# linchaobao/EPPM

Measured on AMD Instinct MI355X. Metric: Mflow-vectors/sec, higher is better.
Workload: dtype f32; 1 GPU; single 1024x436 Sintel-shape synthetic pair per step, full 3-level pyramid, patch_r=9, default defs.h parameters; 1 rank(s), independent pairs; inputs: RGBA planes resident in HBM before the timed region; outputs: interleaved float2 flow left in HBM (the PCIe-inclusive window of the reference API -- host RGB in, host u/v out -- is `host_boundary`, with --full); inputs=device-resident RGBA, outputs=device-resident float2 flow, pairs_in_flight_per_gpu=24, pairs_per_launch=8, contexts_in_flight=3, width=1024, height=436

## Files before the change

eppm_amd/csrc/c2f_device.cuh:

```cuda
#pragma once
#include "eppm_device.cuh"

#ifndef EPPM_C2F_UNROLL
#define EPPM_C2F_UNROLL 2
#endif
#ifndef EPPM_C2F_WAVES
#define EPPM_C2F_WAVES 4
#endif
#ifndef EPPM_C2F_WAVES_MIN
#define EPPM_C2F_WAVES_MIN 2
#endif
#define EPPM_C2F_OCC __attribute__((amdgpu_waves_per_eu(EPPM_C2F_WAVES_MIN, EPPM_C2F_WAVES)))
#ifndef EPPM_C2F_WIN_H
#ifdef EPPM_TOL
#define EPPM_C2F_WIN_H 50
#else
#define EPPM_C2F_WIN_H 48
#endif
#endif
#ifndef EPPM_C2F_PASS2
#define EPPM_C2F_PASS2 1
#endif
#ifndef EPPM_C2F_WIN_WAVES
#define EPPM_C2F_WIN_WAVES 4
#endif
#ifndef EPPM_C2F_PRE
#define EPPM_C2F_PRE 1
#endif
#ifndef EPPM_C2F_PRE_ROWS
#define EPPM_C2F_PRE_ROWS 5
#endif
#ifndef EPPM_C2F_PRE_EPS
#define EPPM_C2F_PRE_EPS 0x1p-13f
#endif
#define EPPM_C2F_PRE_DMIN 0x1p-60f
#define EPPM_C2F_PRE_RHSMIN 0x1p-100f
#ifndef EPPM_C2F_SPLIT_BELOW_WAVES
#define EPPM_C2F_SPLIT_BELOW_WAVES 1024
#endif
#ifndef EPPM_C2F_WINDOW
#define EPPM_C2F_WINDOW 1
#endif
#ifndef EPPM_C2F_WINDOW17
#define EPPM_C2F_WINDOW17 1
#endif
#ifdef EPPM_TOL
#define EPPM_C2F_LOG2 true
#else
#define EPPM_C2F_LOG2 false
#endif
#define EPPM_PRAGMA_(x) _Pragma(#x)
#define EPPM_UNROLL(n) EPPM_PRAGMA_(unroll n)

namespace eppm {

__device__ __forceinline__ Planes to_dev(const PlanesH& h, size_t pstride = 0, unsigned pair = 0)
{
    Planes p;
    p.pk1 = pair_ptr((const float4*)h.pk1, pstride, pair); p.pk2 = pair_ptr((const float4*)h.pk2, pstride, pair);
    p.w = h.w; p.h = h.h; p.pitch = h.pitch;
    return p;
}

__device__ __forceinline__ float4 stage_texel(const uint32_t* __restrict__ pc, const float4* __restrict__ pk, unsigned idx)
{
    if (pc) { const uint32_t w = pc[idx]; return make_texel(w, w >> 24); }
    return pk[idx];
}

__device__ __forceinline__ bool c2f_unknown(float fvx, float fvy) { return fvx > kUnknownFlowThresh || fvy > kUnknownFlowThresh; }
__device__ __forceinline__ int c2f_centre(float f, int x) { return (int)(int16_t)(f2short(f) + x); }
__device__ __forceinline__ void c2f_store_flow(float* flow, int idx, int fx, int fy)
{
    flow[idx * 2] = (float)fx;
    flow[idx * 2 + 1] = (float)fy;
}
__device__ __forceinline__ float c2f_min(float a, float b) { return (a < b) ? a : b; }
__device__ __forceinline__ float c2f_min4(float c1, float c2, float c3, float c4) { return c2f_min(c1, c2f_min(c2, c2f_min(c3, c4))); }
template <class F>
__device__ __forceinline__ void c2f_select_best(float* flow, int x, int y, int ccx, int ccy, int w, int h, F cost_of)
{
    int bx = ccx, by = ccy;
    float min_cost = 999999;
#pragma unroll
    for (int m = 0; m < 3; m++) {
        const int cx = (int)(int16_t)(ccx + m - 1);
        if (cx < 0 || cx >= w) continue;
#pragma unroll
        for (int n = 0; n < 3; n++) {
            const int cy = (int)(int16_t)(ccy + n - 1);
            if (cy < 0 || cy >= h) continue;
            const float cv = cost_of(m, n);
            if (cv < min_cost) { min_cost = cv; bx = cx; by = cy; }
        }
    }
    flow[(y * w + x) * 2] = (float)(bx - x);
    flow[(y * w + x) * 2 + 1] = (float)(by - y);
}

template <int SPLIT>
__device__ __forceinline__ bool c2f_tile_origin(const Planes& P, int& x0, int& y0, int& part)
{
    const int tiles_x = (P.w + kBlock - 1) / kBlock, tiles = tiles_x * ((P.h + kBlock - 1) / kBlock);
    const int per_xcd = (tiles + 7) / 8;
    const int slot = SPLIT ? (blockIdx.x >> 3) / SPLIT : (blockIdx.x >> 3);
    part = SPLIT ? (blockIdx.x >> 3) % SPLIT : -1;
    const int tile = (blockIdx.x & 7) * per_xcd + slot;
    if (slot >= per_xcd || tile >= tiles) return false;
    x0 = (tile % tiles_x) * kBlock; y0 = (tile / tiles_x) * kBlock;
    return true;
}

template <int R> struct C2fSrcTile { static constexpr int TWU = kBlock + 2 * R, TW = (TWU + 15) / 16 * 16; };
template <int R> struct C2fPreList {
    static constexpr int PADB = (C2fSrcTile<R>::TW - C2fSrcTile<R>::TWU) * 16, KROWS = PADB ? (256 * 8 + PADB - 1) / PADB : 0;
    static constexpr int CAP = PADB ? (C2fSrcTile<R>::TWU - KROWS) * (PADB / 2) : 0;
// ... 298 lines not shown
```

eppm_amd/csrc/eppm_internal.h:

```cpp
#pragma once

#include <hip/hip_runtime.h>
#include <stddef.h>
#include <stdint.h>

#include <atomic>

#include "../../include/eppm.h"

namespace eppm {

constexpr int kMaxLevels = 8;
constexpr int kNumLevels = 3;
constexpr int kBlock = 16;
constexpr int kMaxS = 32;
constexpr int kWmfRadius = 4;
constexpr int kBlfRadius = 10;
constexpr int kDeltaSlots = 800;

struct Batch {
    int n;
    size_t stride;
};
constexpr Batch kOnePair = {1, 0};
// ... 57 lines not shown
    int npairs = 1;
    size_t stride = 0;
    size_t cache_plane = 0;
    int wl_units = 0;
    int sweep_seq = 0;
    size_t seed_plane = 0;
    int merged_it = 0;
    int seg_len = 0, nseg_row = 0, nseg_col = 0;
};
int pm_worklist_units(int w, int h, int seg_len);
inline size_t pm_worklist_words(int w, int h, int seg_len) { return 16 + 10 * (size_t)pm_worklist_units(w, h, seg_len); }
struct PmRngDev {
    const uint32_t* init_tab;
    const uint32_t* iter_tab;
    const uint32_t* skip_mat;
    uint32_t skip_weyl;
    int per_lane;
    int gx, gy;
    const int16_t* rand_tab = nullptr;
};
void launch_pm_rand_table(const PmRngDev& rng, uint32_t* work, int16_t* tab, int G, hipStream_t s);
void launch_pm_init_field(const PmBatch& b, const PmRngDev& rng, hipStream_t s);
void launch_pm_cost_field(const PmBatch& b, const float* lut, int R, hipStream_t s);
int pm_parity_kernels(int R);
bool launch_pm_sweep(PmBatch& b, const float* lut, int R, int seg_len, int dir, hipStream_t s, bool speculative = false);
bool launch_pm_sweeps_merged(PmBatch& b, const float* lut, int R, int seg_len, int iteration, hipStream_t s);
void launch_pm_jump(const PmBatch& b, const float* lut, int R, int step, hipStream_t s);
void launch_pm_neighbor(const PmBatch& b, const float* lut, int R, hipStream_t s);
void launch_pm_random_search(const PmBatch& b, const PmRngDev& rng, const float* lut, int R, int search_range, int num_guess,
                             hipStream_t s, bool pretest = false);
void launch_pm_rest_weight(const PmBatch& b, const float* lut, int R, hipStream_t s);
bool pm_search_pretest_ready(const PmBatch& b, const PmRngDev& rng, int R);
struct PmPretestSums { float* n[2]; float* d[2]; };
void launch_pm_pretest_probe(const PmBatch& b, const float* lut, int R, const PmPretestSums& out, hipStream_t s);
EPPM_DECISION bool pm_search_pretest_form(int w, int h, int R, int problems, int npairs);
EPPM_DECISION bool pm_search_pretest(int iteration, int w, int h, int R, int problems, int npairs);
EPPM_DECISION void pm_search_pretest_knobs(int R, int* row0, int* rows, int* from, float* eps);
EPPM_DECISION int pm_search_rows(int w, int h, int R, int problems, int npairs, bool table);
struct SweepForm { int lpc; bool small, pre, tile; };
EPPM_DECISION SweepForm pm_sweep_form(int w, int h, int R, int seg_len, int dir, int problems, int npairs);

struct PmSeed {
    const int16_t* prior[2];
    int16_t* nnf_init[2];
    float* cost_init[2];
    size_t stride = 0;
};
void launch_pm_cost_select(const PmBatch& b, const PmSeed& seed, const float* lut, int R, hipStream_t s);

constexpr int kTemporalMaxSlots = 4096;
struct TemporalArgs {
    const int16_t* prev[2];
    int16_t* prior[2];
    int32_t* keys[2];
    int step[2];
    int w, h, ndir;
    int nslots;
    size_t stride;
    uint32_t armed[kTemporalMaxSlots / 32];
};
void launch_temporal_keys_init(int32_t* keys, int n, hipStream_t s);
void launch_temporal_splat(const TemporalArgs& a, hipStream_t s);
void launch_temporal_gather(const TemporalArgs& a, hipStream_t s);
void launch_temporal_snapshot(int16_t* prev, size_t prev_stride, const int16_t* nnf, int nnf_pitch, int w, int h, hipStream_t s, Batch bt = kOnePair);
void launch_nnf2flow_snapshot(float* flow, int flow_pitch, int16_t* prev, size_t prev_stride, const int16_t* nnf, int nnf_pitch, int w, int h,
                              hipStream_t s, Batch bt = kOnePair);

void launch_lr_check(int16_t* nnf1, float* cost1, const int16_t* nnf2, int w, int h, int cost_pitch, int nnf_pitch, hipStream_t s, Batch bt = kOnePair);
void launch_outlier(int16_t* nnf_out, float* cost, const int16_t* nnf_in, int w, int h, int cost_pitch, int nnf_pitch, hipStream_t s, Batch bt = kOnePair);
size_t wmf_workspace_words(int w, int h, int num_iter);
int16_t* launch_wmf(int16_t* buf_a, int16_t* buf_b, const uint32_t* img, int ipitch, int w, int h, int nnf_pitch,
                    const float* wmf_lut, int num_iter, int only_occlusion, uint32_t* ws, hipStream_t s, Batch bt = kOnePair);
void launch_fill_holes(int16_t* nnf_out, const int16_t* nnf_in, const uint32_t* img, int ipitch, int w, int h, int nnf_pitch,
                       hipStream_t s, Batch bt = kOnePair);
void launch_nnf2flow(float* flow, int flow_pitch, const int16_t* nnf, int nnf_pitch, int w, int h, hipStream_t s, Batch bt = kOnePair);

void launch_resize_flow(float* out, int outH, int outW, const float* in, int h, int w, float ratio, float post_scale, hipStream_t s, Batch bt = kOnePair);
void launch_mul_scalar(float* flow, float scale, int h, int w, hipStream_t s);
EPPM_DECISION int c2f_refine_split_factor(int w, int h, int R, int npairs = 1, bool no_split = false);
bool c2f_refine_wants_split(int w, int h, int R, int npairs = 1, bool no_split = false);
bool c2f_window_span(int R, int* span_x, int* span_y);
void launch_c2f_refine(const PlanesH& P, float* flow, const float* lut, int R, float* cost9, hipStream_t s, Batch bt = kOnePair, bool no_split = false,
                       int pre = -1, unsigned* stat = nullptr, float* probe = nullptr);
void c2f_pretest_knobs(int R, int* on, int* row0, int* rows, int* cap, float* eps, float* dmin, float* rhsmin);
void launch_flow_blf(float* out, const float* in, const uint32_t* img, int ipitch, int w, int h, int flow_pitch,
                     const float* blf_lut, hipStream_t s, Batch bt = kOnePair);
EPPM_DECISION int flow_blf_pixels_per_lane(int w, int h, int npairs = 1);
void launch_flow_jbu(float* out, const float* in_coarse, const uint32_t* img, int ipitch, int w, int h, int wc, int hc, const float* blf_lut,
                     hipStream_t s, Batch bt = kOnePair);

void launch_split_flow(float* uv, const float* flow, int n, hipStream_t s, Batch bt = kOnePair);

void launch_fb_occlusion(uint8_t* occ1, uint8_t* occ2, const float* fwd, size_t fwd_stride, const float* bwd, size_t bwd_stride, int h, int w,
                         float alpha, float beta, int npairs, int ndir, hipStream_t s);

constexpr int kInterpChunk = 4;
struct InterpArgs {
    const uint8_t* img1;
    const uint8_t* img2;
    size_t img_pitch, img_stride;
    const float* flow;
    size_t flow_stride;
    const uint8_t* occ1;
    const uint8_t* occ2;
    size_t occ_stride;
    uint64_t* keys;
    int32_t* fill1;
    int32_t* fill2;
    size_t plane;
    uint8_t* rgb;
    uint8_t* rgba[kInterpChunk];
    size_t rgba_pitch;
    int h, w, nt;
    float t[kInterpChunk];
};
void launch_interp_splat(const InterpArgs& a, int npairs, hipStream_t s);
void launch_interp_fill(const InterpArgs& a, int npairs, hipStream_t s);
void launch_interp_blend(const InterpArgs& a, int npairs, hipStream_t s);

struct MBlurArgs {
    const uint8_t* img;
    size_t img_pitch, img_stride;
    const float* flow;
    size_t flow_stride;
    uint32_t* packed;
    uint64_t* tkeys;
    size_t plane, tplane;
    uint8_t* rgb;
    uint8_t* rgba;
    size_t rgba_pitch;
    int h, w, tiles_x, tiles_y;
    float shutter, max_radius;
    int taps;
};
void launch_mblur_pack(const MBlurArgs& a, int npairs, hipStream_t s);
void launch_mblur_gather(const MBlurArgs& a, int npairs, hipStream_t s);

enum {
    kTrackCntLive, kTrackCntNextId, kTrackCntFrame, kTrackCntDropped, kTrackCntEnded, kTrackCntSeeded,
    kTrackCntIdBase, kTrackCntSurv, kTrackCntPrevLive, kTrackCntSeeded0, kTrackCntDropped0, kTrackCntN = 16
};
struct TrackRec;
struct TrackDev {
    struct {
        int spacing;
        long long min_eig;
        float fb_alpha, fb_beta, mb_alpha, mb_beta;
    } p;
    int cap, ncells, ncx;
    float* npos;
    uint8_t* stat;
    TrackRec* ended;
    int32_t* ended_reason;
    uint8_t* cov;
    uint8_t* flags;
    int32_t *blk_s, *blk_e;
    int32_t* blk_c;
    int32_t* cnt;
};
struct TrackIn {
    const uint8_t* img1;
    const uint8_t* img2;
    size_t pitch;
    const float* fwd;
    const float* bwd;
    int h, w;
};
// ... 195 lines not shown
```

eppm_amd/csrc/k_c2f_refine.hip:

```cpp
#include <type_traits>

#include "c2f_device.cuh"
#include "eppm_internal.h"

namespace eppm {

__constant__ C2fTables<9> c2f_tab9 = make_c2f_tables<9>();
__constant__ C2fTables<17> c2f_tab17 = make_c2f_tables<17>();
template <> __device__ __forceinline__ const C2fTables<9>& c2f_tables<9>() { return c2f_tab9; }
template <> __device__ __forceinline__ const C2fTables<17>& c2f_tables<17>() { return c2f_tab17; }

__global__ __launch_bounds__(256) void k_c2f_refine(PlanesH Ph, float* __restrict__ flow_, const float* __restrict__ lut, int R, size_t pstride)
{
    __shared__ EPPM_LUT_ALIGN PatchLut L;
    load_patch_lut(L, lut, R, threadIdx.y * kBlock + threadIdx.x, 256);
    __syncthreads();
    const Planes P = to_dev(Ph, pstride, blockIdx.z);
    float* __restrict__ flow = pair_ptr(flow_, pstride, blockIdx.z);
    const int x = blockIdx.x * kBlock + threadIdx.x, y = blockIdx.y * kBlock + threadIdx.y;
    if (x >= P.w || y >= P.h) return;
    const float fvx = flow[(y * P.w + x) * 2], fvy = flow[(y * P.w + x) * 2 + 1];
    if (c2f_unknown(fvx, fvy)) { c2f_store_flow(flow, y * P.w + x, 0, 0); return; }
    const int ccx = c2f_centre(fvx, x), ccy = c2f_centre(fvy, y);
    int bx = ccx, by = ccy;
// ... 19 lines not shown
{
    float* __restrict__ flow = pair_ptr(flow_, pstride, blockIdx.y);
    float* __restrict__ cost9 = pair_ptr_opt(cost9_, pstride, blockIdx.y);
    constexpr int TWU = C2fSrcTile<R>::TWU, TW = C2fSrcTile<R>::TW;
    __shared__ EPPM_LUT_ALIGN PatchLutT<R + 1> L;
    __shared__ float4 s_src[TWU * TW];
    const int tid = threadIdx.y * kBlock + threadIdx.x;
    load_patch_lut<EPPM_C2F_LOG2>(L, lut, R, tid, 256);
    const Planes P = to_dev(Ph, pstride, blockIdx.y);
    int x0, y0, part;
    if (!c2f_tile_origin<SPLIT>(P, x0, y0, part)) return;
    const int m_only = (SPLIT == 3) ? part : -1;
    for (int t = tid; t < TWU * TWU; t += 256) {
        const int ry = t / TWU, rx = t % TWU;
        const int sy = iclamp(y0 + ry - R, 0, P.h - 1), sx = iclamp(x0 + rx - R, 0, P.w - 1);
        s_src[ry * TW + rx] = P.pk1[(unsigned)(sy * P.pitch + sx)];
    }
    __syncthreads();
    const int x = x0 + threadIdx.x, y = y0 + threadIdx.y;
    if (x >= P.w || y >= P.h) return;
    const float fvx = flow[(y * P.w + x) * 2], fvy = flow[(y * P.w + x) * 2 + 1];
    if (c2f_unknown(fvx, fvy)) {
        if (SPLIT == 0) c2f_store_flow(flow, y * P.w + x, 0, 0);
        return;
    }
    const int ccx = c2f_centre(fvx, x), ccy = c2f_centre(fvy, y);
    const rgbf c1 = texel_rgb(s_src[(threadIdx.y + R) * TW + threadIdx.x + R]);
    int bx = ccx, by = ccy;
    float min_cost = 999999;
#pragma unroll 1
    for (int m = 0; m < 3; m++) {
        if (SPLIT == 3 && m != m_only) continue;
        const int cx = (int)(int16_t)(ccx + m - 1);
        if (cx < 0 || cx >= P.w) continue;
        rgbf c2[3];
#pragma unroll
        for (int n = 0; n < 3; n++) c2[n] = texel_rgb(tex_px(P.pk2, P.pitch, P.w, P.h, cx, ccy + n - 1));
        float run[3];
        const int cx16 = cx << 4, wmax16 = (P.w - 1) << 4;
        if (SPLIT == 4) {
            if (part == 3) c2f_pass<R, 3, true>(P, L, s_src, TW, threadIdx.x, threadIdx.y, cx16, wmax16, ccy, c1, c2, run);
            else if (part == 2) c2f_pass<R, 2, true>(P, L, s_src, TW, threadIdx.x, threadIdx.y, cx16, wmax16, ccy, c1, c2, run);
            else if (part == 1) c2f_pass<R, 1, true>(P, L, s_src, TW, threadIdx.x, threadIdx.y, cx16, wmax16, ccy, c1, c2, run);
            else c2f_pass<R, 0, true>(P, L, s_src, TW, threadIdx.x, threadIdx.y, cx16, wmax16, ccy, c1, c2, run);
#pragma unroll
            for (int n = 0; n < 3; n++) cost9[(size_t)(y * P.w + x) * 36 + part * 9 + m * 3 + n] = run[n];
            continue;
        }
        c2f_pass<R, 3>(P, L, s_src, TW, threadIdx.x, threadIdx.y, cx16, wmax16, ccy, c1, c2, run);
        c2f_pass<R, 2>(P, L, s_src, TW, threadIdx.x, threadIdx.y, cx16, wmax16, ccy, c1, c2, run);
        c2f_pass<R, 1>(P, L, s_src, TW, threadIdx.x, threadIdx.y, cx16, wmax16, ccy, c1, c2, run);
        c2f_pass<R, 0>(P, L, s_src, TW, threadIdx.x, threadIdx.y, cx16, wmax16, ccy, c1, c2, run);
        if (SPLIT == 3) {
#pragma unroll
            for (int n = 0; n < 3; n++) cost9[(size_t)(y * P.w + x) * 36 + m * 3 + n] = run[n];
            continue;
        }
#pragma unroll
        for (int n = 0; n < 3; n++) {
            const int cy = (int)(int16_t)(ccy + n - 1);
            if (cy < 0 || cy >= P.h) continue;
            const float cv = run[n];
            if (cv < min_cost) { min_cost = cv; bx = cx; by = cy; }
        }
    }
    if (SPLIT != 0) return;
    flow[(y * P.w + x) * 2] = (float)(bx - x);
    flow[(y * P.w + x) * 2 + 1] = (float)(by - y);
}

template <int R, bool PROBE = false>
__global__ __launch_bounds__(512) __attribute__((amdgpu_waves_per_eu(EPPM_C2F_WIN_WAVES, EPPM_C2F_WIN_WAVES)))
void k_c2f_refine_win(PlanesH Ph, float* __restrict__ flow_, const float* __restrict__ lut, size_t pstride, int pre, unsigned* __restrict__ stat,
                      float* __restrict__ probe)
{
    using W = C2fWinShape<R>;
    constexpr int TWU = C2fSrcTile<R>::TWU, TW = C2fSrcTile<R>::TW, WW = W::WW, WH = W::WH;
    static_assert(TWU * TW * 16 >= 9 * 256 * 4, "the exchange buffer aliases the source tile");
    __shared__ EPPM_LUT_ALIGN PatchLutT<R + 1> L;
    __shared__ float4 s_src[TWU * TW];
    __shared__ float4 s_win[WH * WW];
    __shared__ int s_mm[4];
#ifndef EPPM_TOL
    __shared__ int s_pre[8];
#endif
    float* __restrict__ flow = pair_ptr(flow_, pstride, blockIdx.y);
    const int ptid = threadIdx.y * kBlock + threadIdx.x;
    const int grp = threadIdx.z;
    const int tid = grp * 256 + ptid;
    load_patch_lut<EPPM_C2F_LOG2>(L, lut, R, tid, 512);
    const Planes P = to_dev(Ph, pstride, blockIdx.y);
    const uint32_t* __restrict__ pc1 = pair_ptr_opt(Ph.pc1, pstride, blockIdx.y);
    const uint32_t* __restrict__ pc2 = pair_ptr_opt(Ph.pc2, pstride, blockIdx.y);
    int x0, y0, part;
    if (!c2f_tile_origin<0>(P, x0, y0, part)) return;
    if (tid == 0) { s_mm[0] = 0x7fffffff; s_mm[1] = -0x7fffffff; s_mm[2] = 0x7fffffff; s_mm[3] = -0x7fffffff; }
#ifndef EPPM_TOL
    if (tid < 8) s_pre[tid] = 0;
#endif
    for (int t = tid; t < TWU * TWU; t += 512) {
        const int ry = t / TWU, rx = t % TWU;
        const int sy = iclamp(y0 + ry - R, 0, P.h - 1), sx = iclamp(x0 + rx - R, 0, P.w - 1);
        s_src[ry * TW + rx] = stage_texel(pc1, P.pk1, (unsigned)(sy * P.pitch + sx));
    }
    __syncthreads();
    const int x = x0 + threadIdx.x, y = y0 + threadIdx.y;
    const bool inimg = (x < P.w && y < P.h);
    float fvx = 0.0f, fvy = 0.0f;
    if (inimg) { fvx = flow[(y * P.w + x) * 2]; fvy = flow[(y * P.w + x) * 2 + 1]; }
    const bool known = inimg && !(fvx > kUnknownFlowThresh || fvy > kUnknownFlowThresh);
    const int ccx = c2f_centre(fvx, x), ccy = c2f_centre(fvy, y);
    if (known && grp == 0) {
        atomicMin(&s_mm[0], ccx); atomicMax(&s_mm[1], ccx);
        atomicMin(&s_mm[2], ccy); atomicMax(&s_mm[3], ccy);
    }
    __syncthreads();
    const int mnx = s_mm[0], mxx = s_mm[1], mny = s_mm[2], mxy = s_mm[3];
    const bool coherent = (mxx - mnx <= W::SPAN_X) && (mxy - mny <= W::SPAN_Y);
    const int wx0 = mnx - 1 + W::XLO, wy0 = mny - 1 + W::YLO;
    if (coherent && mxx >= mnx) {
        for (int t = tid; t < WH * WW; t += 512) {
            const int sy = iclamp(wy0 + t / WW, 0, P.h - 1), sx = iclamp(wx0 + t % WW, 0, P.w - 1);
            s_win[t] = stage_texel(pc2, P.pk2, (unsigned)(sy * P.pitch + sx));
        }
    }
    __syncthreads();
#ifndef EPPM_TOL
    int path = 3;
    if (pre && coherent && mxx >= mnx) {
        constexpr int S = R + 1, I0 = (S - EPPM_C2F_PRE_ROWS) / 2, I1 = I0 + EPPM_C2F_PRE_ROWS;
        constexpr int PADB = C2fPreList<R>::PADB, KROWS = C2fPreList<R>::KROWS, CAP = C2fPreList<R>::CAP;
        static_assert(PADB % 8 == 0 && PADB > 0 && KROWS < TWU, "keys and items do not straddle a row's padding");
        auto pad = [&](int o) -> char* { return reinterpret_cast<char*>(s_src) + (o / PADB) * (TW * 16) + TWU * 16 + (o % PADB); };
        auto key_at = [&](int p) -> unsigned long long* { return reinterpret_cast<unsigned long long*>(pad(p * 8)); };
        auto item_at = [&](int i) -> uint16_t* { return reinterpret_cast<uint16_t*>(pad(KROWS * PADB + i * 2)); };
        const int lane = tid & 63;
        float N[18], D[18], U = 0.0f;
        unsigned vmask = 0;
        rgbf c1 = {0.0f, 0.0f, 0.0f};
        if (known) {
            c1 = texel_rgb(s_src[(threadIdx.y + R) * TW + threadIdx.x + R]);
#pragma unroll 1
            for (int ii = 0; ii < S; ii++) {
                if (ii >= I0 && ii < I1) continue;
                const float4* __restrict__ srow = s_src + (threadIdx.y + 2 * ii) * TW + threadIdx.x;
#pragma unroll
                for (int jj = 0; jj < S; jj++) U += rest_weight_term(c1, srow[2 * jj], L.gsp[ii * S + jj]);
            }
        }
#pragma unroll
        for (int m = 0; m < 3; m++) {
            const int cx = (int)(int16_t)(ccx + m - 1);
            float cs[6] = {0.0f, 0.0f, 0.0f, 0.0f, 0.0f, 0.0f}, ws[6] = {0.0f, 0.0f, 0.0f, 0.0f, 0.0f, 0.0f};
            if (known && !(cx < 0 || cx >= P.w)) {
                const int wbase = ((ccy - 1 - wy0) * WW + (cx - wx0)) * 16;
                rgbf c2[3];
#pragma unroll
                for (int n = 0; n < 3; n++) {
                    c2[n] = texel_rgb(*reinterpret_cast<const float4*>(reinterpret_cast<const char*>(s_win) + wbase + n * (WW * 16)));
                    const int cy = (int)(int16_t)(ccy + n - 1);
                    if (!(cy < 0 || cy >= P.h)) vmask |= 1u << (m * 3 + n);
                }
                if (grp == 0) c2f_rows2_win<R, 3, 2, WW, I0, I1, 3>(L, s_src, TW, threadIdx.x, threadIdx.y, c1, c2, s_win, wbase, cs, ws);
                else c2f_rows2_win<R, 1, 0, WW, I0, I1, 3>(L, s_src, TW, threadIdx.x, threadIdx.y, c1, c2, s_win, wbase, cs, ws);
            }
#pragma unroll
            for (int n = 0; n < 3; n++) { N[m * 3 + n] = cs[n]; D[m * 3 + n] = ws[n]; N[9 + m * 3 + n] = cs[3 + n]; D[9 + m * 3 + n] = ws[3 + n]; }
        }
        if (PROBE && known) {
            float* __restrict__ pp = probe + ((size_t)blockIdx.y * P.h * P.w + (size_t)y * P.w + x) * 73;
            const int qa = (grp == 0 ? 3 : 1) * 9, qb = (grp == 0 ? 2 : 0) * 9;
#pragma unroll
            for (int k = 0; k < 9; k++) { pp[qa + k] = N[k]; pp[36 + qa + k] = D[k]; pp[qb + k] = N[9 + k]; pp[36 + qb + k] = D[9 + k]; }
            if (grp == 1) pp[72] = U;
        }
        bool small = false;
#pragma unroll
        for (int k = 0; k < 9; k++)
            if ((vmask >> k) & 1) small = small || !(D[k] > EPPM_C2F_PRE_DMIN) || !(D[9 + k] > EPPM_C2F_PRE_DMIN);
        if (small) s_pre[0] = 1;
        if (grp == 1) {
            int ks = 15;
            float e_best = 0.0f;
#pragma unroll
            for (int k = 0; k < 9; k++) {
                if (!((vmask >> k) & 1)) continue;
                const float e = c2f_min(N[k] / D[k], N[9 + k] / D[9 + k]);
                if (ks == 15 || e < e_best) { e_best = e; ks = k; }
            }
            *key_at(ptid) = 0xfffffffffffffff0ull | (unsigned)ks;
        }
        __syncthreads();
        path = 1;
        if (!s_pre[0]) {
            const int ks = (int)(*reinterpret_cast<const uint32_t*>(key_at(ptid)) & 15u);
            const bool live = known && ks != 15;
            if (live) {
                const int cx = (int)(int16_t)(ccx + ks / 3 - 1);
                const int wbase = ((ccy - 1 + ks % 3 - wy0) * WW + (cx - wx0)) * 16;
                const rgbf c2[1] = {texel_rgb(*reinterpret_cast<const float4*>(reinterpret_cast<const char*>(s_win) + wbase))};
                float cs[2], ws[2];
                if (grp == 0) c2f_rows2_win<R, 3, 2, WW, 0, S, 1>(L, s_src, TW, threadIdx.x, threadIdx.y, c1, c2, s_win, wbase, cs, ws);
                else c2f_rows2_win<R, 1, 0, WW, 0, S, 1>(L, s_src, TW, threadIdx.x, threadIdx.y, c1, c2, s_win, wbase, cs, ws);
                const float c = c2f_min(cs[0] / ws[0], cs[1] / ws[1]);
                atomicMin(key_at(ptid), ((unsigned long long)__float_as_uint(c) << 4) | (unsigned)ks);
            }
            __syncthreads();
            unsigned sa = 0, sb = 0, tested = 0;
            if (live) {
                const float B = __uint_as_float((uint32_t)(*key_at(ptid) >> 4));
#pragma unroll
                for (int k = 0; k < 9; k++) {
                    if (!((vmask >> k) & 1) || k == ks) continue;
                    const float ra = B * (D[k] + U), rb = B * (D[9 + k] + U);
                    if (!(N[k] * (1.0f - EPPM_C2F_PRE_EPS) >= ra && ra >= EPPM_C2F_PRE_RHSMIN)) sa |= 1u << k;
                    if (!(N[9 + k] * (1.0f - EPPM_C2F_PRE_EPS) >= rb && rb >= EPPM_C2F_PRE_RHSMIN)) sb |= 1u << k;
                    tested += 2;
                }
            }
            const int na = __popc(sa), nb = __popc(sb);
            int ia = na, ib = nb;
#pragma unroll
            for (int d = 1; d < 64; d <<= 1) {
                const int ta = __shfl_up(ia, d), tb = __shfl_up(ib, d);
                if (lane >= d) { ia += ta; ib += tb; }
            }
            const int pa = grp == 0 ? 3 : 1, pb = grp == 0 ? 2 : 0;
            int wa = 0, wb = 0;
            if (lane == 63) { wa = atomicAdd(&s_pre[1 + pa], ia); wb = atomicAdd(&s_pre[1 + pb], ib); }
            wa = __shfl(wa, 63); wb = __shfl(wb, 63);
            if (stat && tested) { atomicAdd(stat + 4, tested); atomicAdd(stat + 5, tested - (unsigned)(na + nb)); }
            __syncthreads();
            int cnt[4], chb[5];
            chb[0] = 0;
#pragma unroll
            for (int p = 0; p < 4; p++) { cnt[p] = s_pre[1 + p]; chb[p + 1] = chb[p] + ((cnt[p] + 63) >> 6); }
            path = 2;
            if (chb[4] * 64 <= CAP) {
                path = 0;
                {
                    int at = chb[pa] * 64 + wa + ia - na;
                    for (unsigned s = sa; s; s &= s - 1) *item_at(at++) = (uint16_t)(ptid | ((__ffs(s) - 1) << 8));
                    at = chb[pb] * 64 + wb + ib - nb;
                    for (unsigned s = sb; s; s &= s - 1) *item_at(at++) = (uint16_t)(ptid | ((__ffs(s) - 1) << 8));
                }
                __syncthreads();
                for (int c = tid >> 6; c < chb[4]; c += 8) {
                    const int p = __builtin_amdgcn_readfirstlane((c >= chb[1]) + (c >= chb[2]) + (c >= chb[3]));
                    const int idx = (c - chb[p]) * 64 + lane;
                    if (idx < cnt[p]) {
                        const unsigned it = *item_at(chb[p] * 64 + idx);
                        const int ip = it & 255, k = it >> 8, tx = ip & (kBlock - 1), ty = ip / kBlock;
                        const int px = x0 + tx, py = y0 + ty;
                        const int qcx = c2f_centre(flow[(py * P.w + px) * 2], px), qcy = c2f_centre(flow[(py * P.w + px) * 2 + 1], py);
                        const int cx = (int)(int16_t)(qcx + k / 3 - 1);
                        const int wbase = ((qcy - 1 + k % 3 - wy0) * WW + (cx - wx0)) * 16;
                        const rgbf q1 = texel_rgb(s_src[(ty + R) * TW + tx + R]);
                        const rgbf q2 = texel_rgb(*reinterpret_cast<const float4*>(reinterpret_cast<const char*>(s_win) + wbase));
                        float c_;
                        if (p == 3) c_ = c2f_one_win<R, 3, WW>(L, s_src, TW, tx, ty, q1, q2, s_win, wbase);
                        else if (p == 2) c_ = c2f_one_win<R, 2, WW>(L, s_src, TW, tx, ty, q1, q2, s_win, wbase);
                        else if (p == 1) c_ = c2f_one_win<R, 1, WW>(L, s_src, TW, tx, ty, q1, q2, s_win, wbase);
                        else c_ = c2f_one_win<R, 0, WW>(L, s_src, TW, tx, ty, q1, q2, s_win, wbase);
                        atomicMin(key_at(ip), ((unsigned long long)__float_as_uint(c_) << 4) | (unsigned)k);
                    }
                }
                __syncthreads();
                if (stat && tid == 0) atomicAdd(stat + 0, 1u);
                if (grp != 1 || !inimg) return;
                if (!known) { c2f_store_flow(flow, y * P.w + x, 0, 0); return; }
                int k = (int)(*key_at(ptid) & 15u);
                if (k == 15) k = 4;
                c2f_store_flow(flow, y * P.w + x, (int)(int16_t)(ccx + k / 3 - 1) - x, (int)(int16_t)(ccy + k % 3 - 1) - y);
                return;
            }
        }
    }
    if (stat && tid == 0) atomicAdd(stat + path, 1u);
#endif
    float res[9];
    float res1[9];
    if (known) {
        const rgbf c1 = texel_rgb(s_src[(threadIdx.y + R) * TW + threadIdx.x + R]);
#pragma unroll
        for (int m = 0; m < 3; m++) {
            const int cx = (int)(int16_t)(ccx + m - 1);
            float run[3] = {0.0f, 0.0f, 0.0f}, raw[3] = {0.0f, 0.0f, 0.0f};
            if (!(cx < 0 || cx >= P.w)) {
                rgbf c2[3];
                const int cx16 = cx << 4, wmax16 = (P.w - 1) << 4;
                if (coherent) {
                    const int wbase = ((ccy - 1 - wy0) * WW + (cx - wx0)) * 16;
#pragma unroll
                    for (int n = 0; n < 3; n++) c2[n] = texel_rgb(*reinterpret_cast<const float4*>(reinterpret_cast<const char*>(s_win) + wbase + n * (WW * 16)));
#if EPPM_C2F_PASS2
                    if (grp == 0) {
                        float c4[3], c3[3];
                        c2f_pass2_win<R, 3, 2, WW>(L, s_src, TW, threadIdx.x, threadIdx.y, c1, c2, s_win, wbase, c4, c3);
#pragma unroll
                        for (int n = 0; n < 3; n++) run[n] = c2f_min(c3[n], c4[n]);
                    } else {
                        c2f_pass2_win<R, 1, 0, WW>(L, s_src, TW, threadIdx.x, threadIdx.y, c1, c2, s_win, wbase, run, raw);
                    }
#else
                    if (grp == 0) {
                        c2f_pass<R, 3, false, true, WW>(P, L, s_src, TW, threadIdx.x, threadIdx.y, cx16, wmax16, ccy, c1, c2, run, s_win, wbase);
                        c2f_pass<R, 2, false, true, WW>(P, L, s_src, TW, threadIdx.x, threadIdx.y, cx16, wmax16, ccy, c1, c2, run, s_win, wbase);
                    } else {
                        c2f_pass<R, 1, true, true, WW>(P, L, s_src, TW, threadIdx.x, threadIdx.y, cx16, wmax16, ccy, c1, c2, run, s_win, wbase);
                        c2f_pass<R, 0, true, true, WW>(P, L, s_src, TW, threadIdx.x, threadIdx.y, cx16, wmax16, ccy, c1, c2, raw, s_win, wbase);
                    }
#endif
                } else {
#pragma unroll
                    for (int n = 0; n < 3; n++) c2[n] = texel_rgb(tex_px(P.pk2, P.pitch, P.w, P.h, cx, ccy + n - 1));
                    if (grp == 0) {
                        c2f_pass<R, 3>(P, L, s_src, TW, threadIdx.x, threadIdx.y, cx16, wmax16, ccy, c1, c2, run);
                        c2f_pass<R, 2>(P, L, s_src, TW, threadIdx.x, threadIdx.y, cx16, wmax16, ccy, c1, c2, run);
                    } else {
                        c2f_pass<R, 1, true>(P, L, s_src, TW, threadIdx.x, threadIdx.y, cx16, wmax16, ccy, c1, c2, run);
                        c2f_pass<R, 0, true>(P, L, s_src, TW, threadIdx.x, threadIdx.y, cx16, wmax16, ccy, c1, c2, raw);
                    }
                }
            }
#pragma unroll
            for (int n = 0; n < 3; n++) { res[m * 3 + n] = run[n]; res1[m * 3 + n] = raw[n]; }
        }
    }
    __syncthreads();
    float* __restrict__ xch = reinterpret_cast<float*>(s_src);
    if (grp == 0 && known) {
#pragma unroll
        for (int k = 0; k < 9; k++) xch[k * 256 + ptid] = res[k];
    }
    __syncthreads();
    if (grp != 1 || !inimg) return;
    if (!known) { c2f_store_flow(flow, y * P.w + x, 0, 0); return; }
    int bx = ccx, by = ccy;
    float min_cost = 999999;
#pragma unroll
    for (int m = 0; m < 3; m++) {
        const int cx = (int)(int16_t)(ccx + m - 1);
        if (cx < 0 || cx >= P.w) continue;
#pragma unroll
        for (int n = 0; n < 3; n++) {
            const int cy = (int)(int16_t)(ccy + n - 1);
            if (cy < 0 || cy >= P.h) continue;
            const float m34 = xch[(m * 3 + n) * 256 + ptid];
            const float c_2 = res[m * 3 + n], c_1 = res1[m * 3 + n];
            const float cv = c2f_min(c_1, c2f_min(c_2, m34));
            if (cv < min_cost) { min_cost = cv; bx = cx; by = cy; }
// ... 63 lines not shown
            if (!(cx < 0 || cx >= P.w)) {
                rgbf c2[3];
                const int cx16 = cx << 4, wmax16 = (P.w - 1) << 4;
                if (coherent) {
                    const int wbase = ((ccy - 1 - wy0) * WW + (cx - wx0)) * 16;
#pragma unroll
                    for (int n = 0; n < 3; n++) c2[n] = texel_rgb(*reinterpret_cast<const float4*>(reinterpret_cast<const char*>(s_win) + wbase + n * (WW * 16)));
                    if (grp == 0) c2f_pass<R, 3, true, true, WW>(P, L, s_src, TW, threadIdx.x, threadIdx.y, cx16, wmax16, ccy, c1, c2, run, s_win, wbase);
                    else if (grp == 1) c2f_pass<R, 2, true, true, WW>(P, L, s_src, TW, threadIdx.x, threadIdx.y, cx16, wmax16, ccy, c1, c2, run, s_win, wbase);
                    else if (grp == 2) c2f_pass<R, 1, true, true, WW>(P, L, s_src, TW, threadIdx.x, threadIdx.y, cx16, wmax16, ccy, c1, c2, run, s_win, wbase);
                    else c2f_pass<R, 0, true, true, WW>(P, L, s_src, TW, threadIdx.x, threadIdx.y, cx16, wmax16, ccy, c1, c2, run, s_win, wbase);
                } else {
#pragma unroll
                    for (int n = 0; n < 3; n++) c2[n] = texel_rgb(tex_px(P.pk2, P.pitch, P.w, P.h, cx, ccy + n - 1));
                    if (grp == 0) c2f_pass<R, 3, true>(P, L, s_src, TW, threadIdx.x, threadIdx.y, cx16, wmax16, ccy, c1, c2, run);
                    else if (grp == 1) c2f_pass<R, 2, true>(P, L, s_src, TW, threadIdx.x, threadIdx.y, cx16, wmax16, ccy, c1, c2, run);
                    else if (grp == 2) c2f_pass<R, 1, true>(P, L, s_src, TW, threadIdx.x, threadIdx.y, cx16, wmax16, ccy, c1, c2, run);
                    else c2f_pass<R, 0, true>(P, L, s_src, TW, threadIdx.x, threadIdx.y, cx16, wmax16, ccy, c1, c2, run);
                }
            }
#pragma unroll
            for (int n = 0; n < 3; n++) res[m * 3 + n] = run[n];
        }
    }
    __syncthreads();
    float* __restrict__ xch = reinterpret_cast<float*>(s_src);
    if (grp != 0 && known) {
#pragma unroll
        for (int k = 0; k < 9; k++) xch[((grp - 1) * 9 + k) * 256 + ptid] = res[k];
    }
    __syncthreads();
    if (grp != 0 || !inimg) return;
    if (!known) { c2f_store_flow(flow, y * P.w + x, 0, 0); return; }
    int bx = ccx, by = ccy;
    float min_cost = 999999;
#pragma unroll
    for (int m = 0; m < 3; m++) {
        const int cx = (int)(int16_t)(ccx + m - 1);
        if (cx < 0 || cx >= P.w) continue;
#pragma unroll
        for (int n = 0; n < 3; n++) {
            const int cy = (int)(int16_t)(ccy + n - 1);
            if (cy < 0 || cy >= P.h) continue;
            const int k = m * 3 + n;
            const float c_4 = res[k], c_3 = xch[k * 256 + ptid], c_2 = xch[(9 + k) * 256 + ptid], c_1 = xch[(18 + k) * 256 + ptid];
            const float cv = c2f_min4(c_1, c_2, c_3, c_4);
            if (cv < min_cost) { min_cost = cv; bx = cx; by = cy; }
        }
    }
    flow[(y * P.w + x) * 2] = (float)(bx - x);
    flow[(y * P.w + x) * 2 + 1] = (float)(by - y);
}

template <int SPLIT>
__global__ __launch_bounds__(256) void k_c2f_select(float* __restrict__ flow_, const float* __restrict__ cost9_, int w, int h, size_t pstride)
{
    float* __restrict__ flow = pair_ptr(flow_, pstride, blockIdx.z);
    const float* __restrict__ cost9 = pair_ptr(cost9_, pstride, blockIdx.z);
    const int x = blockIdx.x * blockDim.x + threadIdx.x, y = blockIdx.y * blockDim.y + threadIdx.y;
    if (x >= w || y >= h) return;
    const float fvx = flow[(y * w + x) * 2], fvy = flow[(y * w + x) * 2 + 1];
    if (c2f_unknown(fvx, fvy)) { c2f_store_flow(flow, y * w + x, 0, 0); return; }
    c2f_select_best(flow, x, y, c2f_centre(fvx, x), c2f_centre(fvy, y), w, h, [=](int m, int n) {
        const float* __restrict__ pc = cost9 + (size_t)(y * w + x) * 36 + m * 3 + n;
        float cv = pc[0];
        if (SPLIT == 4) {
            cv = pc[27];
            cv = c2f_min(pc[18], cv);
            cv = c2f_min(pc[9], cv);
            cv = c2f_min(pc[0], cv);
        }
        return cv;
    });
}

bool c2f_window_span(int R, int* span_x, int* span_y)
{
    if (!(R == 9 || R == 17)) return false;
    *span_x = (R == 9) ? C2fWinShape<9>::SPAN_X : C2fWinShape<17>::SPAN_X;
    *span_y = (R == 9) ? C2fWinShape<9>::SPAN_Y : C2fWinShape<17>::SPAN_Y;
    return true;
}

void c2f_pretest_knobs(int R, int* on, int* row0, int* rows, int* cap, float* eps, float* dmin, float* rhsmin)
{
#ifdef EPPM_TOL
    *on = 0;
#else
    *on = EPPM_C2F_PRE;
#endif
    *row0 = (R + 1 - EPPM_C2F_PRE_ROWS) / 2; *rows = EPPM_C2F_PRE_ROWS;
    *cap = C2fPreList<9>::CAP;
    *eps = EPPM_C2F_PRE_EPS; *dmin = EPPM_C2F_PRE_DMIN; *rhsmin = EPPM_C2F_PRE_RHSMIN;
}

static bool c2f_table_ok(int w, int h, int R) { return (w + R < 32764) && (h + R < 32764); }

int c2f_refine_split_factor(int w, int h, int R, int npairs, bool no_split)
{
    if (no_split || !(R == 9 || R == 17) || !c2f_table_ok(w, h, R)) return 0;
    const int tiles = ((w + kBlock - 1) / kBlock) * ((h + kBlock - 1) / kBlock);
    if (!(tiles * npairs * 4 < EPPM_C2F_SPLIT_BELOW_WAVES)) return 0;
    auto imbalance = [&](int f) { const int wgs = tiles * f * npairs; return (float)((wgs + 255) / 256) * 256.0f / (float)wgs; };
    return (imbalance(4) < imbalance(3)) ? 4 : 3;
}
bool c2f_refine_wants_split(int w, int h, int R, int npairs, bool no_split) { return c2f_refine_split_factor(w, h, R, npairs, no_split) != 0; }

template <class F>
static void with_radius(int R, F&& f)
{
    if (R == 9) f(std::integral_constant<int, 9>{});
    else f(std::integral_constant<int, 17>{});
}

void launch_c2f_refine(const PlanesH& P, float* flow, const float* lut, int R, float* cost9, hipStream_t s, Batch bt, bool no_split, int pre,
                       unsigned* stat, float* probe)
{
    dim3 grid((P.w + kBlock - 1) / kBlock, (P.h + kBlock - 1) / kBlock, bt.n), block(kBlock, kBlock);
    const int per_xcd = (grid.x * grid.y + 7) / 8;
    dim3 grid1(per_xcd * 8, bt.n);
    const int f = cost9 ? c2f_refine_split_factor(P.w, P.h, R, bt.n, no_split) : 0;
    launch_note(kLaunchRefine, P.w, P.h, bt.n, f, R);
    if (f) {
        dim3 gridf(per_xcd * f * 8, bt.n), gs((P.w + 63) / 64, (P.h + 3) / 4, bt.n), bs(64, 4);
        with_radius(R, [&](auto r) {
            if (f == 3) hipLaunchKernelGGL((k_c2f_refine_tiled<r(), 3>), gridf, block, 0, s, P, flow, lut, cost9, bt.stride);
            else hipLaunchKernelGGL((k_c2f_refine_tiled<r(), 4>), gridf, block, 0, s, P, flow, lut, cost9, bt.stride);
        });
        if (f == 3) hipLaunchKernelGGL(k_c2f_select<3>, gs, bs, 0, s, flow, cost9, P.w, P.h, bt.stride);
        else hipLaunchKernelGGL(k_c2f_select<4>, gs, bs, 0, s, flow, cost9, P.w, P.h, bt.stride);
        return;
    }
    if (!(R == 9 || R == 17) || !c2f_table_ok(P.w, P.h, R)) {
        hipLaunchKernelGGL(k_c2f_refine, grid, block, 0, s, P, flow, lut, R, bt.stride);
        return;
    }
    const bool window = (R == 9) ? EPPM_C2F_WINDOW : EPPM_C2F_WINDOW17;
    if (!window) with_radius(R, [&](auto r) { hipLaunchKernelGGL((k_c2f_refine_tiled<r(), 0>), grid1, block, 0, s, P, flow, lut, (float*)nullptr, bt.stride); });
    else if (R == 9 && probe) hipLaunchKernelGGL((k_c2f_refine_win<9, true>), grid1, dim3(kBlock, kBlock, 2), 0, s, P, flow, lut, bt.stride, 1, stat, probe);
    else if (R == 9) hipLaunchKernelGGL((k_c2f_refine_win<9>), grid1, dim3(kBlock, kBlock, 2), 0, s, P, flow, lut, bt.stride, pre < 0 ? EPPM_C2F_PRE : pre, stat, (float*)nullptr);
    else hipLaunchKernelGGL((k_c2f_refine_win4<17>), grid1, dim3(kBlock, kBlock, 4), 0, s, P, flow, lut, bt.stride);
}

}
```

eppm_amd/stages.py:

```python
import ctypes as C

import numpy as np

from ._lib import CParams, check, check_launcher, lib, probe_dispatch
from .api import float2, short2, uchar4


class Dev:

    def __init__(self, arr=None, shape=None, dtype=None, pitched=False):
        if arr is not None:
            arr = np.ascontiguousarray(arr)
            shape, dtype = arr.shape, arr.dtype
        self.h, self.w = shape
        self.dtype = np.dtype(dtype)
        row = self.w * self.dtype.itemsize
        self.ptr = C.c_void_p()
        if pitched:
            pitch = C.c_size_t()
            check(lib().eppm_malloc_pitched(C.byref(self.ptr), C.byref(pitch), C.c_size_t(row), C.c_size_t(self.h)), "malloc_pitched")
            self.pitch = pitch.value
        else:
            check(lib().eppm_malloc_device(C.byref(self.ptr), C.c_size_t(row * self.h)), "malloc")
            self.pitch = row
# ... 196 lines not shown
    check(lib().eppm_probe_search_pretest(iteration, w, h, patch_r, problems, npairs, out, C.byref(eps)), "eppm_probe_search_pretest")
    return bool(out[0]), out[1], out[2], out[3], eps.value, bool(out[4])


def patchmatch(P):
    n, c = Dev(shape=(P.h, P.w), dtype=short2), Dev(shape=(P.h, P.w), dtype=np.float32)
    lib().baoCudaPatchMatch(n.ptr, c.ptr, *P.args(), P.w, P.h, _sz(P.i1.pitch), _sz(c.pitch), _sz(n.pitch), _sz(P.c1.pitch))
    check_launcher("baoCudaPatchMatch")
    return n.get(), c.get()


def left_right_check(nnf1, cost1, nnf2, cost2):
    h, w = nnf1.shape
    a, b, c, d = Dev(nnf1), Dev(cost1), Dev(nnf2), Dev(cost2)
    lib().baoCudaLeftRightCheck(a.ptr, b.ptr, c.ptr, d.ptr, w, h, _sz(b.pitch), _sz(a.pitch))
    check_launcher("baoCudaLeftRightCheck")
    return a.get(), b.get(), c.get(), d.get()


def outlier_removal(nnf, cost):
    h, w = nnf.shape
    a, b = Dev(nnf), Dev(cost)
    lib().baoCudaOutlierRemoval(a.ptr, b.ptr, w, h, _sz(b.pitch), _sz(a.pitch))
    check_launcher("baoCudaOutlierRemoval")
    return a.get(), b.get()


def weighted_median(nnf, img, num_iter=20, only_occlusion=True):
    h, w = nnf.shape
    a, i = Dev(nnf), Dev(img, pitched=True)
    lib().baoCudaWeightedMedianFilter(a.ptr, None, i.ptr, w, h, _sz(i.pitch), _sz(w * 4), _sz(a.pitch), num_iter, C.c_bool(only_occlusion))
    check_launcher("baoCudaWeightedMedianFilter")
    return a.get()


def fill_holes(nnf, img):
    h, w = nnf.shape
    a, i = Dev(nnf), Dev(img, pitched=True)
    lib().baoCudaFillHole(a.ptr, None, i.ptr, w, h, _sz(i.pitch), _sz(w * 4), _sz(a.pitch))
    check_launcher("baoCudaFillHole")
    return a.get()


def nnf2flow(nnf):
    h, w = nnf.shape
    a, f = Dev(nnf), Dev(shape=(h, w), dtype=float2)
    lib().baoCudaNNF2Flow(f.ptr, a.ptr, w, h, _sz(a.pitch), _sz(f.pitch))
    check_launcher("baoCudaNNF2Flow")
    return f.get()


def resize_flow(flow, out_h, out_w, ratio=2.0):
    h, w = flow.shape
    a, b = Dev(flow), Dev(shape=(out_h, out_w), dtype=float2)
    check(lib().eppm_resize_flow(b.ptr, out_h, out_w, a.ptr, h, w, C.c_float(ratio)), "resize_flow")
    return b.get()


def flow_upsample(coarse, img):
    h, w = img.shape
    hc, wc = coarse.shape
    a, i, b = Dev(coarse), Dev(img, pitched=True), Dev(shape=(h, w), dtype=float2)
    check(lib().eppm_flow_upsample(b.ptr, h, w, a.ptr, hc, wc, i.ptr, _sz(i.pitch)), "eppm_flow_upsample")
    return b.get()


def c2f_refine(flow, P):
    f = Dev(flow)
    lib().baoCudaBLFCostFilterRefine(f.ptr, *P.args(), P.w, P.h, _sz(P.i1.pitch), _sz(P.c1.pitch))
    check_launcher("baoCudaBLFCostFilterRefine")
    return f.get()


def c2f_refine_batch(flows, planes):
    n = len(flows)
    h, w = flows[0].shape
    f = Dev(np.concatenate([np.ascontiguousarray(x, float2) for x in flows]))
    i1, i2, c1, c2 = (Dev(np.concatenate([np.ascontiguousarray(p[k]) for p in planes])) for k in range(4))
    check(lib().eppm_test_c2f_refine_batch(f.ptr, i1.ptr, i2.ptr, c1.ptr, c2.ptr, w, h, n), "eppm_test_c2f_refine_batch")
    out = f.get()
    return [out[k * h:(k + 1) * h] for k in range(n)]


def c2f_refine_pre(flows, planes, pre):
    n = len(flows)
    h, w = flows[0].shape
    f = Dev(np.concatenate([np.ascontiguousarray(x, float2) for x in flows]))
    i1, i2, c1, c2 = (Dev(np.concatenate([np.ascontiguousarray(p[k]) for p in planes])) for k in range(4))
    stat = (C.c_uint * 8)()
    check(lib().eppm_test_c2f_refine_pre(f.ptr, i1.ptr, i2.ptr, c1.ptr, c2.ptr, w, h, n, int(pre), stat), "eppm_test_c2f_refine_pre")
    out = f.get()
    return [out[k * h:(k + 1) * h] for k in range(n)], tuple(stat[:6])


def c2f_refine_probe(flows, planes):
    n = len(flows)
    h, w = flows[0].shape
    f = Dev(np.concatenate([np.ascontiguousarray(x, float2) for x in flows]))
    i1, i2, c1, c2 = (Dev(np.concatenate([np.ascontiguousarray(p[k]) for p in planes])) for k in range(4))
    pr = Dev(shape=(n * h, w * 73), dtype=np.float32)
    check(lib().eppm_test_c2f_refine_probe(f.ptr, i1.ptr, i2.ptr, c1.ptr, c2.ptr, w, h, n, pr.ptr), "eppm_test_c2f_refine_probe")
    out, p = f.get(), pr.get().reshape(n, h, w, 73)
    return [out[k * h:(k + 1) * h] for k in range(n)], p[..., :36].reshape(n, h, w, 4, 9), p[..., 36:72].reshape(n, h, w, 4, 9), p[..., 72]


def probe_c2f_pretest(patch_r=9):
    out = (C.c_int * 4)()
    fl = (C.c_float * 3)()
    check(lib().eppm_probe_c2f_pretest(patch_r, out, fl), "eppm_probe_c2f_pretest")
    return bool(out[0]), out[1], out[2], out[3], fl[0], fl[1], fl[2]


def blf_c2f(flow_coarse, P_fine, coarse_dims):
    ch, cw = coarse_dims
    fine = Dev(shape=(P_fine.h, P_fine.w), dtype=float2)
    coarse = Dev(flow_coarse)
    tab = lambda a, b: (C.c_void_p * 2)(a, b)
    arrH = (C.c_int * 2)(P_fine.h, ch)
    arrW = (C.c_int * 2)(P_fine.w, cw)
    p4 = (C.c_size_t * 2)(P_fine.i1.pitch, 0)
    pc = (C.c_size_t * 2)(P_fine.c1.pitch, 0)
    lib().baoCudaBLF_C2F(tab(fine.ptr, coarse.ptr), tab(P_fine.i1.ptr, None), tab(P_fine.i2.ptr, None), tab(P_fine.c1.ptr, None),
                         tab(P_fine.c2.ptr, None), None, None, arrH, arrW, p4, pc, 0)
    check_launcher("baoCudaBLF_C2F")
    return fine.get()


def flow_smoothing(flow, img):
    h, w = flow.shape
    f, i = Dev(flow), Dev(img, pitched=True)
    lib().baoCudaFlowSmoothing(f.ptr, i.ptr, w, h, _sz(i.pitch), _sz(f.pitch))
    check_launcher("baoCudaFlowSmoothing")
    return f.get()


def temporal_prior(prev, backward=False):
    d_prev = Dev(np.ascontiguousarray(prev, short2))
    d_out = Dev(shape=prev.shape, dtype=short2)
    check(lib().eppm_temporal_prior(d_out.ptr, d_prev.ptr, d_prev.h, d_prev.w, int(bool(backward))), "eppm_temporal_prior")
    check(lib().eppm_device_synchronize(), "eppm_device_synchronize")
    return d_out.get()


def temporal_prior_batch(prevs, backward=False, armed=None, calls=1):
    prevs = np.ascontiguousarray(prevs, short2)
    n, h, w = prevs.shape
    d_prev = Dev(prevs.reshape(n * h, w))
    d_out = Dev(shape=(n * h, w), dtype=short2)
    flags = None if armed is None else (C.c_uint8 * n)(*[int(bool(x)) for x in armed])
    out = []
    for _ in range(calls):
        check(lib().eppm_temporal_prior_batch(d_out.ptr, d_prev.ptr, h, w, int(bool(backward)), n, flags), "eppm_temporal_prior_batch")
        check(lib().eppm_device_synchronize(), "eppm_device_synchronize")
        out.append(d_out.get().reshape(n, h, w))
    return out[0] if calls == 1 else out


def flow_to_color(flow, max_disp_x=20.0, max_disp_y=20.0):
    h, w = flow.shape
    f, c = Dev(flow), Dev(shape=(h, w), dtype=uchar4)
    check(lib().eppm_flow_to_color(c.ptr, f.ptr, h, w, C.c_float(max_disp_x), C.c_float(max_disp_y)), "eppm_flow_to_color")
    return c.get()
```

Baseline: 256.3 Mflow-vectors/s.

## Split overflowing c2f pretest candidate list into per-quarter passes

Per-wave candidate counts now go to shared scratch instead of shared atomics, and each wave works out its list offsets from those counts. When the combined candidate list would exceed the list capacity, the tile is processed in halves or quarters, each filling and draining the list in turn. This keeps such tiles on the cheap candidate-list path rather than falling back to the full evaluation path. It adds extra barriers and a loop per part.

```diff
diff --git a/eppm_amd/csrc/c2f_device.cuh b/eppm_amd/csrc/c2f_device.cuh
--- a/eppm_amd/csrc/c2f_device.cuh
+++ b/eppm_amd/csrc/c2f_device.cuh
@@ -32,6 +32,9 @@
 #endif
 #ifndef EPPM_C2F_PRE_EPS
 #define EPPM_C2F_PRE_EPS 0x1p-13f
+#endif
+#ifndef EPPM_C2F_PRE_PARTS
+#define EPPM_C2F_PRE_PARTS 1
 #endif
 #define EPPM_C2F_PRE_DMIN 0x1p-60f
 #define EPPM_C2F_PRE_RHSMIN 0x1p-100f
diff --git a/eppm_amd/csrc/eppm_internal.h b/eppm_amd/csrc/eppm_internal.h
--- a/eppm_amd/csrc/eppm_internal.h
+++ b/eppm_amd/csrc/eppm_internal.h
@@ -163,7 +163,7 @@
 bool c2f_window_span(int R, int* span_x, int* span_y);
 void launch_c2f_refine(const PlanesH& P, float* flow, const float* lut, int R, float* cost9, hipStream_t s, Batch bt = kOnePair, bool no_split = false,
                        int pre = -1, unsigned* stat = nullptr, float* probe = nullptr);
-void c2f_pretest_knobs(int R, int* on, int* row0, int* rows, int* cap, float* eps, float* dmin, float* rhsmin);
+void c2f_pretest_knobs(int R, int* on, int* row0, int* rows, int* cap, int* parts, float* eps, float* dmin, float* rhsmin);
 void launch_flow_blf(float* out, const float* in, const uint32_t* img, int ipitch, int w, int h, int flow_pitch,
                      const float* blf_lut, hipStream_t s, Batch bt = kOnePair);
 EPPM_DECISION int flow_blf_pixels_per_lane(int w, int h, int npairs = 1);
diff --git a/eppm_amd/csrc/k_c2f_refine.hip b/eppm_amd/csrc/k_c2f_refine.hip
--- a/eppm_amd/csrc/k_c2f_refine.hip
+++ b/eppm_amd/csrc/k_c2f_refine.hip
@@ -125,7 +125,7 @@
     __shared__ float4 s_win[WH * WW];
     __shared__ int s_mm[4];
 #ifndef EPPM_TOL
-    __shared__ int s_pre[8];
+    __shared__ int s_pre[1];
 #endif
     float* __restrict__ flow = pair_ptr(flow_, pstride, blockIdx.y);
     const int ptid = threadIdx.y * kBlock + threadIdx.x;
@@ -139,7 +139,7 @@
     if (!c2f_tile_origin<0>(P, x0, y0, part)) return;
     if (tid == 0) { s_mm[0] = 0x7fffffff; s_mm[1] = -0x7fffffff; s_mm[2] = 0x7fffffff; s_mm[3] = -0x7fffffff; }
 #ifndef EPPM_TOL
-    if (tid < 8) s_pre[tid] = 0;
+    if (tid == 0) s_pre[0] = 0;
 #endif
     for (int t = tid; t < TWU * TWU; t += 512) {
         const int ry = t / TWU, rx = t % TWU;
@@ -268,48 +268,86 @@
                 const int ta = __shfl_up(ia, d), tb = __shfl_up(ib, d);
                 if (lane >= d) { ia += ta; ib += tb; }
             }
-            const int pa = grp == 0 ? 3 : 1, pb = grp == 0 ? 2 : 0;
-            int wa = 0, wb = 0;
-            if (lane == 63) { wa = atomicAdd(&s_pre[1 + pa], ia); wb = atomicAdd(&s_pre[1 + pb], ib); }
-            wa = __shfl(wa, 63); wb = __shfl(wb, 63);
+            static_assert(KROWS * PADB >= 256 * 8 + 16 * 4, "the counts follow the keys");
+            auto qcnt_at = [&](int i) -> int* { return reinterpret_cast<int*>(pad(256 * 8 + i * 4)); };
+            const int wq = __builtin_amdgcn_readfirstlane((tid >> 6) & 3);
+            if (lane == 63) { *qcnt_at(wq * 4 + (grp == 0 ? 3 : 1)) = ia; *qcnt_at(wq * 4 + (grp == 0 ? 2 : 0)) = ib; }
             if (stat && tested) { atomicAdd(stat + 4, tested); atomicAdd(stat + 5, tested - (unsigned)(na + nb)); }
             __syncthreads();
-            int cnt[4], chb[5];
-            chb[0] = 0;
-#pragma unroll
-            for (int p = 0; p < 4; p++) { cnt[p] = s_pre[1 + p]; chb[p + 1] = chb[p] + ((cnt[p] + 63) >> 6); }
+            int qc[4][4];
+#pragma unroll
+            for (int q = 0; q < 4; q++)
+#pragma unroll
+                for (int p = 0; p < 4; p++) qc[q][p] = __builtin_amdgcn_readfirstlane(*qcnt_at(q * 4 + p));
+            auto chunks_of = [&](int qlo, int qhi) {
+                int c = 0;
+#pragma unroll
+                for (int p = 0; p < 4; p++) {
+                    int s = 0;
+#pragma unroll
+                    for (int q = 0; q < 4; q++) s += (q >= qlo && q < qhi) ? qc[q][p] : 0;
+                    c += (s + 63) >> 6;
+                }
+                return c;
+            };
+            static_assert(64 * 8 * 4 <= CAP, "a quarter of the tile always fits the list");
+            int qw = 4;
+            if (chunks_of(0, 4) * 64 > CAP) qw = (chunks_of(0, 2) * 64 <= CAP && chunks_of(2, 4) * 64 <= CAP) ? 2 : 1;
             path = 2;
-            if (chb[4] * 64 <= CAP) {
-                path = 0;
-                {
-                    int at = chb[pa] * 64 + wa + ia - na;
-                    for (unsigned s = sa; s; s &= s - 1) *item_at(at++) = (uint16_t)(ptid | ((__ffs(s) - 1) << 8));
-                    at = chb[pb] * 64 + wb + ib - nb;
-                    for (unsigned s = sb; s; s &= s - 1) *item_at(at++) = (uint16_t)(ptid | ((__ffs(s) - 1) << 8));
+            if (qw == 4 || EPPM_C2F_PRE_PARTS) {
+                const int ba = ia - na, bb = ib - nb;
+#pragma unroll 1
+                for (int qlo = 0; qlo < 4; qlo += qw) {
+                    const int qhi = qlo + qw;
+                    int cnt[4], chb[5];
+                    chb[0] = 0;
+#pragma unroll
+                    for (int p = 0; p < 4; p++) {
+                        int s = 0;
+#pragma unroll
+                        for (int q = 0; q < 4; q++) s += (q >= qlo && q < qhi) ? qc[q][p] : 0;
+                        cnt[p] = s; chb[p + 1] = chb[p] + ((s + 63) >> 6);
+                    }
+                    if (wq >= qlo && wq < qhi) {
+                        int oa = 0, ob = 0;
+#pragma unroll
+                        for (int q = 0; q < 3; q++) {
+                            const bool before = (q >= qlo && q < wq);
+                            oa += before ? (grp == 0 ? qc[q][3] : qc[q][1]) : 0;
+                            ob += before ? (grp == 0 ? qc[q][2] : qc[q][0]) : 0;
+                        }
+                        int at = (grp == 0 ? chb[3] : chb[1]) * 64 + oa + ba;
+                        for (unsigned s = sa; s; s &= s - 1) *item_at(at++) = (uint16_t)(ptid | ((__ffs(s) - 1) << 8));
+                        at = (grp == 0 ? chb[2] : chb[0]) * 64 + ob + bb;
+                        for (unsigned s = sb; s; s &= s - 1) *item_at(at++) = (uint16_t)(ptid | ((__ffs(s) - 1) << 8));
+                    }
+                    __syncthreads();
+                    for (int c = tid >> 6; c < chb[4]; c += 8) {
+                        const int p = __builtin_amdgcn_readfirstlane((c >= chb[1]) + (c >= chb[2]) + (c >= chb[3]));
+                        const int idx = (c - chb[p]) * 64 + lane;
+                        if (idx < cnt[p]) {
+                            const unsigned it = *item_at(chb[p] * 64 + idx);
+                            const int ip = it & 255, k = it >> 8, tx = ip & (kBlock - 1), ty = ip / kBlock;
+                            const int px = x0 + tx, py = y0 + ty;
+                            const int qcx = c2f_centre(flow[(py * P.w + px) * 2], px), qcy = c2f_centre(flow[(py * P.w + px) * 2 + 1], py);
+                            const int cx = (int)(int16_t)(qcx + k / 3 - 1);
+                            const int wbase = ((qcy - 1 + k % 3 - wy0) * WW + (cx - wx0)) * 16;
+                            const rgbf q1 = texel_rgb(s_src[(ty + R) * TW + tx + R]);
+                            const rgbf q2 = texel_rgb(*reinterpret_cast<const float4*>(reinterpret_cast<const char*>(s_win) + wbase));
+                            float c_;
+                            if (p == 3) c_ = c2f_one_win<R, 3, WW>(L, s_src, TW, tx, ty, q1, q2, s_win, wbase);
+                            else if (p == 2) c_ = c2f_one_win<R, 2, WW>(L, s_src, TW, tx, ty, q1, q2, s_win, wbase);
+                            else if (p == 1) c_ = c2f_one_win<R, 1, WW>(L, s_src, TW, tx, ty, q1, q2, s_win, wbase);
+                            else c_ = c2f_one_win<R, 0, WW>(L, s_src, TW, tx, ty, q1, q2, s_win, wbase);
+                            atomicMin(key_at(ip), ((unsigned long long)__float_as_uint(c_) << 4) | (unsigned)k);
+                        }
+                    }
+                    __syncthreads();
                 }
-                __syncthreads();
-                for (int c = tid >> 6; c < chb[4]; c += 8) {
-                    const int p = __builtin_amdgcn_readfirstlane((c >= chb[1]) + (c >= chb[2]) + (c >= chb[3]));
-                    const int idx = (c - chb[p]) * 64 + lane;
-                    if (idx < cnt[p]) {
-                        const unsigned it = *item_at(chb[p] * 64 + idx);
-                        const int ip = it & 255, k = it >> 8, tx = ip & (kBlock - 1), ty = ip / kBlock;
-                        const int px = x0 + tx, py = y0 + ty;
-                        const int qcx = c2f_centre(flow[(py * P.w + px) * 2], px), qcy = c2f_centre(flow[(py * P.w + px) * 2 + 1], py);
-                        const int cx = (int)(int16_t)(qcx + k / 3 - 1);
-                        const int wbase = ((qcy - 1 + k % 3 - wy0) * WW + (cx - wx0)) * 16;
-                        const rgbf q1 = texel_rgb(s_src[(ty + R) * TW + tx + R]);
-                        const rgbf q2 = texel_rgb(*reinterpret_cast<const float4*>(reinterpret_cast<const char*>(s_win) + wbase));
-                        float c_;
-                        if (p == 3) c_ = c2f_one_win<R, 3, WW>(L, s_src, TW, tx, ty, q1, q2, s_win, wbase);
-                        else if (p == 2) c_ = c2f_one_win<R, 2, WW>(L, s_src, TW, tx, ty, q1, q2, s_win, wbase);
-                        else if (p == 1) c_ = c2f_one_win<R, 1, WW>(L, s_src, TW, tx, ty, q1, q2, s_win, wbase);
-                        else c_ = c2f_one_win<R, 0, WW>(L, s_src, TW, tx, ty, q1, q2, s_win, wbase);
-                        atomicMin(key_at(ip), ((unsigned long long)__float_as_uint(c_) << 4) | (unsigned)k);
-                    }
+                if (stat && tid == 0) {
+                    atomicAdd(stat + (qw == 4 ? 0 : 2), 1u);
+                    if (qw != 4) atomicAdd(stat + (qw == 2 ? 6 : 7), 1u);
                 }
-                __syncthreads();
-                if (stat && tid == 0) atomicAdd(stat + 0, 1u);
                 if (grp != 1 || !inimg) return;
                 if (!known) { c2f_store_flow(flow, y * P.w + x, 0, 0); return; }
                 int k = (int)(*key_at(ptid) & 15u);
@@ -539,7 +577,7 @@
     return true;
 }
 
-void c2f_pretest_knobs(int R, int* on, int* row0, int* rows, int* cap, float* eps, float* dmin, float* rhsmin)
+void c2f_pretest_knobs(int R, int* on, int* row0, int* rows, int* cap, int* parts, float* eps, float* dmin, float* rhsmin)
 {
 #ifdef EPPM_TOL
     *on = 0;
@@ -548,6 +586,7 @@
 #endif
     *row0 = (R + 1 - EPPM_C2F_PRE_ROWS) / 2; *rows = EPPM_C2F_PRE_ROWS;
     *cap = C2fPreList<9>::CAP;
+    *parts = EPPM_C2F_PRE_PARTS;
     *eps = EPPM_C2F_PRE_EPS; *dmin = EPPM_C2F_PRE_DMIN; *rhsmin = EPPM_C2F_PRE_RHSMIN;
 }
 
diff --git a/eppm_amd/stages.py b/eppm_amd/stages.py
--- a/eppm_amd/stages.py
+++ b/eppm_amd/stages.py
@@ -302,7 +302,7 @@
     return [out[k * h:(k + 1) * h] for k in range(n)]
 
 
-def c2f_refine_pre(flows, planes, pre):
+def c2f_refine_pre(flows, planes, pre, parts=False):
     n = len(flows)
     h, w = flows[0].shape
     f = Dev(np.concatenate([np.ascontiguousarray(x, float2) for x in flows]))
@@ -310,7 +310,7 @@
     stat = (C.c_uint * 8)()
     check(lib().eppm_test_c2f_refine_pre(f.ptr, i1.ptr, i2.ptr, c1.ptr, c2.ptr, w, h, n, int(pre), stat), "eppm_test_c2f_refine_pre")
     out = f.get()
-    return [out[k * h:(k + 1) * h] for k in range(n)], tuple(stat[:6])
+    return [out[k * h:(k + 1) * h] for k in range(n)], tuple(stat[:8 if parts else 6])
 
 
 def c2f_refine_probe(flows, planes):
@@ -325,10 +325,19 @@
 
 
 def probe_c2f_pretest(patch_r=9):
-    out = (C.c_int * 4)()
+    out, fl = _c2f_pretest_knobs(patch_r)
+    return bool(out[0]), out[1], out[2], out[3], fl[0], fl[1], fl[2]
+
+
+def probe_c2f_parts(patch_r=9):
+    return bool(_c2f_pretest_knobs(patch_r)[0][4])
+
+
+def _c2f_pretest_knobs(patch_r):
+    out = (C.c_int * 5)()
     fl = (C.c_float * 3)()
     check(lib().eppm_probe_c2f_pretest(patch_r, out, fl), "eppm_probe_c2f_pretest")
-    return bool(out[0]), out[1], out[2], out[3], fl[0], fl[1], fl[2]
+    return out, fl
 
 
 def blf_c2f(flow_coarse, P_fine, coarse_dims):
```

Result: faster. 261.4 Mflow-vectors/s, median of 6 (+2.0%).
